# Kotstantinovskiy/SonicDiffusionBayesLab

Measured on AMD Instinct MI355X. Metric: 512x512 images/sec at 50 DDIM steps, higher is better.
Workload: dtype bf16; 1 GPU; SD-1.5 512x512 DDIM 50 steps, CFG 7.5, batch=8/GPU (BASELINE configs[1]); global_batch=8, sample_size=64, parallelism=batch-shard x1, weights=SD-1.5-shaped synthetic seed 1234

## Files before the change

### sonicdiffusionbayeslab_amd/asm_lint.py

```python
from __future__ import annotations

import re
import sys

_REG = re.compile(r'\b([va])\[(\d+):(\d+)\]|\b([va])(\d+)\b')


def regs(tok: str) -> set:
    out = set()
    for m in _REG.finditer(tok):
        if m.group(1):
            out |= {f"{m.group(1)}{i}" for i in range(int(m.group(2)), int(m.group(3)) + 1)}
        else:
            out.add(f"{m.group(4)}{m.group(5)}")
    return out


def kernels(text: str, want: str = ""):
    for m in re.finditer(r'^(\w+):[ \t]*; @\1[^\n]*\n(.*?)^\.Lfunc_end\d+:', text, flags=re.S | re.M):
        if want in m.group(1):
            yield m.group(1), m.group(2)


def _instructions(body: str):
    for line in body.split("\n"):
        mm = re.match(r'^(\.LBB\d+_\d+):', line)
        if mm:
            yield mm.group(1), None
            continue
        t = line.split(";")[0].strip()
        if t and not t.startswith("."):
            yield None, t


def _split_ops(rest: str):
    out, depth, cur = [], 0, ""
    for ch in rest:
        if ch == "[":
            depth += 1
        elif ch == "]":
            depth -= 1
        if ch == "," and depth == 0:
            out.append(cur.strip()); cur = ""
        else:
            cur += ch
    if cur.strip():
        out.append(cur.strip())
    return out


_PASSES = (("v_mfma_f32_16x16x32_bf16", 4), ("v_mfma_f32_16x16x32_f16", 4), ("v_mfma_f32_16x16x32_fp8", 4), ("v_mfma_f32_16x16x32_bf8", 4),
           ("v_mfma_f32_32x32x16_bf16", 8), ("v_mfma_f32_32x32x16_f16", 8), ("v_mfma_f32_32x32x16_fp8", 8), ("v_mfma_f32_32x32x16_bf8", 8),
           ("v_mfma_scale_f32_16x16x128_f8f6f4", 8), ("v_mfma_f32_16x16x128_f8f6f4", 8),
           ("v_mfma_scale_f32_32x32x64_f8f6f4", 16), ("v_mfma_f32_32x32x64_f8f6f4", 16))


def _mfma_passes(op: str) -> int:
    for name, p in _PASSES:
        if op.startswith(name):
            return p
    return 16


def check_pk_opsel(name: str, body: str):
    errs = []
    for _, t in _instructions(body):
        if t and re.match(r'v_pk_\w+_f32\b', t):
            m = re.search(r'op_sel:\[([01,]+)\]', t)
            if m and "1" in m.group(1):
                errs.append(f"{name}: PK_OPSEL `{t}`")
    return errs


def check_store_soffset(name: str, body: str):
    errs = []
    for _, t in _instructions(body):
        if t and re.match(r'buffer_store_(dwordx3|dwordx4|b96|b128|format_xyzw?)\b', t):
            ops = _split_ops(t.split(None, 1)[1])
            soff = ops[3].split()[0] if len(ops) > 3 else "0"
            if re.match(r's\d+|m0|ttmp', soff):
                errs.append(f"{name}: STORE_SOFF `{t}`")
    return errs


def check_mfma_distance(name: str, body: str):
    errs = []
    live = []
    for lab, t in _instructions(body):
        if t is None:
            continue
        op = t.split()[0]
        rest = t.split(None, 1)[1] if " " in t else ""
        if op in ("s_branch", "s_endpgm", "s_setpc_b64"):
            live = []
            continue
        if op == "s_nop":
            n = int(rest.strip()) + 1
            for e in live:
                e[0] += n
            continue
        ops = _split_ops(rest)
        is_mfma = op.startswith("v_mfma") or op.startswith("v_smfmac")
        reads, writes = set(), set()
        if op.startswith("v_") and not is_mfma:
            if op.startswith(("v_cmp", "v_readfirstlane", "v_readlane")):
                for o in ops[1:]:
                    reads |= regs(o)
            elif op.startswith(("v_swap", "v_permlane16_swap", "v_permlane32_swap")):
                for o in ops:
                    reads |= regs(o); writes |= regs(o)
            else:
                writes |= regs(ops[0]) if ops else set()
                for o in ops[1:]:
                    reads |= regs(o)
                if op.startswith(("v_fmac", "v_mac", "v_pk_fmac", "v_dot2c", "v_accvgpr_write")) and ops:
                    reads |= regs(ops[0])
        elif op.startswith(("ds_write", "ds_store", "buffer_store", "global_store", "flat_store", "scratch_store", "buffer_atomic", "global_atomic")):
            for o in ops:
                reads |= regs(o)
        elif op.startswith(("ds_read", "ds_load", "buffer_load", "global_load", "flat_load", "scratch_load", "ds_bpermute", "ds_permute", "ds_swizzle")):
            if ops and " lds" not in (" " + rest):
                writes |= regs(ops[0])
            for o in ops[1:]:
                reads |= regs(o)
            if " lds" in (" " + rest) and ops:
                reads |= regs(ops[0])
        if not is_mfma:
            for ws, p, d, c, mt in live:
                if reads & d and ws < p + 4:
                    errs.append(f"{name}: MFMA_DIST `{t}` reads {sorted(reads & d)[:2]} {ws} wait states after `{mt}` (needs {p + 4})")
                if writes & d and ws < p + 1:
                    errs.append(f"{name}: MFMA_DIST `{t}` writes {sorted(writes & d)[:2]} {ws} wait states after `{mt}` (needs {p + 1})")
                if writes & c and ws < p - 4:
                    errs.append(f"{name}: MFMA_DIST `{t}` writes SrcC {sorted(writes & c)[:2]} {ws} wait states after `{mt}` (needs {p - 4})")
        for e in live:
            e[0] += 1
        live = [e for e in live if e[0] < 24]
        if is_mfma and len(ops) >= 4:
            d = regs(ops[0]); c = regs(ops[3].split()[0]) - d
            live.append([0, _mfma_passes(op), d, c, t])
    return errs


def check_lds_waits(name: str, body: str):
    errors = []
    blocks, cur, lab = [], [], "entry"
    for l, t in _instructions(body):
        if l:
            blocks.append((lab, cur)); cur = []; lab = l
        else:
            cur.append(t)
    blocks.append((lab, cur))
    n_tr = 0
    for lab, ins in blocks:
        pending = []
        has_tr = any(i.startswith("ds_read_b64_tr_b16") for i in ins)
        for k, i in enumerate(ins):
            op = i.split()[0]
            if op.startswith("scratch_"):
                errors.append(f"{name} {lab}: spill instruction `{i}`")
                continue
            if op.startswith("ds_"):
                touched = regs(i.split(None, 1)[1]) if " " in i else set()
                for _, d in pending:
                    if d & touched:
                        errors.append(f"{name} {lab}: `{i}` names {sorted(d & touched)} while an LDS read into it is in flight")
                dest = regs(i.split(None, 1)[1].split(",")[0]) if op.startswith("ds_read") else set()
                pending.append((op, dest))
                n_tr += op == "ds_read_b64_tr_b16"
                continue
            if op.startswith("s_load") or op.startswith("s_buffer_load") or op == "s_memtime":
                if has_tr:
                    errors.append(f"{name} {lab}: scalar-memory instruction `{i}` in a block with counted LDS waits")
                continue
            if op == "s_waitcnt":
                mm = re.search(r'lgkmcnt\((\d+)\)', i)
                if mm:
                    n = int(mm.group(1))
                    pending = pending[len(pending) - n:] if n else []
                elif "vmcnt" not in i and "expcnt" not in i:
                    pending = []
                continue
            touched = regs(i.split(None, 1)[1]) if " " in i else set()
            for o, d in pending:
                if d & touched:
                    errors.append(f"{name} {lab}: `{i}` (instruction {k}) uses {sorted(d & touched)} before the {o} that writes it is waited for")
        if has_tr and any(o == "ds_read_b64_tr_b16" for o, _ in pending):
            errors.append(f"{name} {lab}: block ends with transposed reads still in flight")
    return errors, n_tr


LDS_WAIT_KERNELS = {"attention": ["attn_pipe40_kernel", "attn_pipe80_kernel", "attn_pipe64_kernel"]}


def lint_file(path: str, unit: str | None = None, verbose: bool = True):
    text = open(path).read()
    unit = unit or path.rsplit("/", 1)[-1].split(".")[0]
    bad, nk = [], 0
    for name, body in kernels(text):
        nk += 1
        bad += check_pk_opsel(name, body)
        bad += check_store_soffset(name, body)
        bad += check_mfma_distance(name, body)
    for want in LDS_WAIT_KERNELS.get(unit, []):
        found = 0
        for name, body in kernels(text, want):
            found += 1
            errs, n_tr = check_lds_waits(name, body)
            if verbose:
                print(f"{name}: {n_tr} ds_read_b64_tr_b16, {len(errs)} violation(s)")
            bad += errs
        if not found:
            bad.append(f"no kernel matching {want} in {path}")
    if nk != text.count(".amdhsa_kernel "):
        bad.append(f"{path}: {text.count('.amdhsa_kernel ')} kernel descriptors but {nk} function bodies recognised")
    if verbose:
        print(f"asm_lint {path}: {nk} kernels, {len(bad)} violation(s)")
        for e in bad[:40]:
            print("  VIOLATION:", e)
    return bad


if __name__ == "__main__":
    rc = 0
    for p in sys.argv[1:]:
        rc |= 1 if lint_file(p) else 0
    sys.exit(rc)
```

### sonicdiffusionbayeslab_amd/csrc/attention.hip

```cpp
#include "common.h"
#include "kernels.h"

#include <stdlib.h>

namespace {

__device__ __forceinline__ float half_pair_max(float x) {
    const unsigned a = __builtin_bit_cast(unsigned, x);
    const auto sw = __builtin_amdgcn_permlane32_swap(a, a, false, false);
    const unsigned r0 = sw[0], r1 = sw[1];
    return fmaxf(__builtin_bit_cast(float, r0), __builtin_bit_cast(float, r1));
}

__device__ __forceinline__ int pi_swap23(int r) { return (r & ~12) | ((r & 4) << 1) | ((r & 8) >> 1); }

__device__ __forceinline__ void xcd_work_item(int nq, int heads, int xcd_order, int& qblk, int& head, int& b) {
    const int G = gridDim.x, L = blockIdx.x;
    const int q = G >> 3, r = G & 7, xcd = L & 7, idx = L >> 3;
    const int v = xcd_order ? (xcd < r ? xcd * (q + 1) : r * (q + 1) + (xcd - r) * q) + idx : L;
    qblk = v % nq;
    const int rest = v / nq;
    head = rest % heads;
    b = rest / heads;
}
// ... 496 lines not shown
    for (int j = 0; j < NIW; ++j) {
        const int inst = wave + NW * j;
        d_ptr[j] = zero; d_step[j] = 0;
        if (inst < CHK) {
            const int ch = inst * 64 + lane, key = ch / CHK, part = ch - key * CHK;
            if (part < CD) {
                const long ld = a.kv_head_major ? D : a.ldk;
                const long base = a.kv_head_major ? ((long)b * a.heads + head) * a.Nk * D : (long)b * a.Nk * a.ldk + head * D;
                d_ptr[j] = (const char*)(a.K + base + (long)key * ld + part * 8);
                d_step[j] = 64 * ld * 2;
            }
        } else if (inst < NI) {
            const int ch = (inst - CHK) * 64 + lane, key = ch / CHV, part = ch - key * CHV;
            if (part < CD) {
                const long ld = a.kv_head_major ? D : a.ldv;
                const long base = a.kv_head_major ? ((long)b * a.heads + head) * a.Nk * D : (long)b * a.Nk * a.ldv + head * D;
                d_ptr[j] = (const char*)(a.V + base + (long)key * ld + part * 8);
                d_step[j] = 64 * ld * 2;
            } else if (part == CD) {
                d_ptr[j] = ones;
            }
        } else if (V & 2) {
            d_ptr[j] = ones;
        }
    }
    const int ntiles = a.Nk / 64;
    auto issue = [&](int t) {
        char* base = smem + (t & 3) * TILE;
        const bool real = t < ntiles;
#pragma unroll
        for (int j = 0; j < NIW; ++j) {
            const char* src = real ? d_ptr[j] + d_step[j] * t : zero;
            glds16(src, base + (wave + NW * j) * 1024);
        }
    };
    auto wait_keep = [&](int tiles_in_flight) {
        if (tiles_in_flight == 2) asm volatile("s_waitcnt vmcnt(%0)" ::"n"(2 * NIW) : "memory");
        else if (tiles_in_flight == 1) asm volatile("s_waitcnt vmcnt(%0)" ::"n"(NIW) : "memory");
        else asm volatile("s_waitcnt vmcnt(0)" ::: "memory");
    };

    f32x16 o[DVT];
#pragma unroll
    for (int t = 0; t < DVT; ++t)
#pragma unroll
        for (int i = 0; i < 16; ++i) o[t][i] = 0.f;

    const int kfrag_off = pi_swap23(r) * RSK + h * 16;
    static_assert(KBYTES + 37 * RSV + 2 * CD * 8 + 32 * RSK >= 11 * 1024 && KBYTES + 37 * RSV + 2 * CD * 8 + 32 * RSK + 16 <= 12 * 1024,
                  "second ones chunk inside the padding piece");
    const int kfrag2_off = h ? KBYTES + 37 * RSV + 2 * CD * 8 - 64 : kfrag_off;
    const int g16 = (lane >> 4) & 1, q4 = (lane & 15) >> 2, p4 = lane & 3;
    const int vtr_off = KBYTES + (8 * h + q4) * RSV + (16 * g16 + 4 * p4) * 2;

    auto qk = [&](const char* tile, f32x16& s0, f32x16& s1) {
        const char* kp = tile + kfrag_off;
        bf16x8 kf[2 * KQ];
#pragma unroll
        for (int kk = 0; kk < KQ; ++kk) {
            const char* kpp = ((V & 2) && kk == KQ - 1) ? tile + kfrag2_off : kp;
            kf[kk] = *(const bf16x8*)(kpp + kk * 32);
            kf[KQ + kk] = *(const bf16x8*)(kpp + 32 * RSK + kk * 32);
        }
        s0 = __builtin_amdgcn_mfma_f32_32x32x16_bf16(kf[0], qf[0], f32x16{}, 0, 0, 0);
        s1 = __builtin_amdgcn_mfma_f32_32x32x16_bf16(kf[KQ], qf[0], f32x16{}, 0, 0, 0);
#pragma unroll
        for (int kk = 1; kk < KQ; ++kk) {
            s0 = __builtin_amdgcn_mfma_f32_32x32x16_bf16(kf[kk], qf[kk], s0, 0, 0, 0);
            s1 = __builtin_amdgcn_mfma_f32_32x32x16_bf16(kf[KQ + kk], qf[kk], s1, 0, 0, 0);
        }
    };
    auto tile_max = [&](const f32x16& s0, const f32x16& s1) -> float {
        float tmax = fmaxf(s0[0], s1[0]);
#pragma unroll
        for (int i = 1; i < 16; ++i) tmax = fmaxf(tmax, fmaxf(s0[i], s1[i]));
        return half_pair_max(tmax);
    };
    auto softmax_p = [&](const f32x16& s0, const f32x16& s1, float mc, bf16x8* pf) {
#pragma unroll
        for (int s2 = 0; s2 < 4; ++s2) {
            float p[8];
#pragma unroll
            for (int j = 0; j < 8; ++j) {
                const float sv = s2 < 2 ? s0[8 * s2 + j] : s1[8 * (s2 - 2) + j];
                p[j] = (V & 2) ? __builtin_amdgcn_exp2f(sv) : __builtin_amdgcn_exp2f(__builtin_fmaf(sv, c, -mc));
            }
            u32x4 w = {pack2bf(p[0], p[1]), pack2bf(p[2], p[3]), pack2bf(p[4], p[5]), pack2bf(p[6], p[7])};
            pf[s2] = __builtin_bit_cast(bf16x8, w);
        }
    };
    auto pv = [&](const char* tile, const bf16x8* pf) {
#pragma unroll
        for (int tt = 0; tt < DVT; ++tt) {
#pragma unroll
            for (int s2 = 0; s2 < 4; ++s2) {
                const char* ap = tile + s2 * 16 * RSV + vtr_off + tt * 64;
                const bf16x4 lo = __builtin_amdgcn_ds_read_tr16_b64_v4i16((__attribute__((address_space(3))) bf16x4*)(ap));
                const bf16x4 hi = __builtin_amdgcn_ds_read_tr16_b64_v4i16((__attribute__((address_space(3))) bf16x4*)(ap + 4 * RSV));
                const bf16x8 vf = bf16x8{lo[0], lo[1], lo[2], lo[3], hi[0], hi[1], hi[2], hi[3]};
                o[tt] = __builtin_amdgcn_mfma_f32_32x32x16_bf16(vf, pf[s2], o[tt], 0, 0, 0);
            }
        }
    };

    issue(0);
    issue(1);
    issue(2);
    wait_keep(2);
    __builtin_amdgcn_s_barrier();
    asm volatile("" ::: "memory");
    f32x16 sa0, sa1, sb0, sb1;
    qk(smem, sa0, sa1);
    float m_run = tile_max(sa0, sa1);
    auto set_ref = [&](float m) -> float {
        const unsigned pb = pack2bf(-m, 0.f) & 0xffffu;
        if (h) qf[KQ - 1][0] = (short)pb;
        return -bf2f((bf16_t)pb);
    };
    if (V & 2) {
        m_run = set_ref(m_run);
#pragma unroll
        for (int i = 0; i < 16; ++i) { sa0[i] -= m_run; sa1[i] -= m_run; }
    }
    constexpr float STALE = 8.f;
    const unsigned lds_v = (unsigned)(size_t)(__attribute__((address_space(3))) char*)smem + (unsigned)vtr_off;

    auto exp_group = [&](const f32x16& c0, const f32x16& c1, int s2, float mc) -> bf16x8 {
        float p[8];
        if (V & 2) {
#pragma unroll
            for (int j = 0; j < 8; ++j) p[j] = __builtin_amdgcn_exp2f(s2 < 2 ? c0[8 * s2 + j] : c1[8 * (s2 - 2) + j]);
            u32x4 w = {pack2bf(p[0], p[1]), pack2bf(p[2], p[3]), pack2bf(p[4], p[5]), pack2bf(p[6], p[7])};
            return __builtin_bit_cast(bf16x8, w);
        }
        const f32x2_t cc = {c, c}, mm = {-mc, -mc};
#pragma unroll
        for (int j = 0; j < 8; j += 2) {
            const f32x2_t sv = s2 < 2 ? f32x2_t{c0[8 * s2 + j], c0[8 * s2 + j + 1]}
                                      : f32x2_t{c1[8 * (s2 - 2) + j], c1[8 * (s2 - 2) + j + 1]};
            const f32x2_t e = __builtin_elementwise_fma(sv, cc, mm);
            p[j] = __builtin_amdgcn_exp2f(e[0]);
            p[j + 1] = __builtin_amdgcn_exp2f(e[1]);
        }
        u32x4 w = {pack2bf(p[0], p[1]), pack2bf(p[2], p[3]), pack2bf(p[4], p[5]), pack2bf(p[6], p[7])};
        return __builtin_bit_cast(bf16x8, w);
    };
    auto vfrag = [&](const char* tile, int tt, int s2) -> bf16x8 {
        const char* ap = tile + s2 * 16 * RSV + vtr_off + tt * 64;
        const bf16x4 lo = __builtin_amdgcn_ds_read_tr16_b64_v4i16((__attribute__((address_space(3))) bf16x4*)(ap));
        const bf16x4 hi = __builtin_amdgcn_ds_read_tr16_b64_v4i16((__attribute__((address_space(3))) bf16x4*)(ap + 4 * RSV));
        return bf16x8{lo[0], lo[1], lo[2], lo[3], hi[0], hi[1], hi[2], hi[3]};
    };
    auto steady = [&](int t, f32x16& c0, f32x16& c1, f32x16& n0, f32x16& n1) {
        wait_keep(1);
        __builtin_amdgcn_s_barrier();
        asm volatile("" ::: "memory");
        issue(t + 3);
        const char* cur = smem + (t & 3) * TILE;
        const char* kp = smem + ((t + 1) & 3) * TILE + kfrag_off;
        const char* kp2 = (V & 2) ? smem + ((t + 1) & 3) * TILE + kfrag2_off : kp;
        const float mc = m_run * c;
        bf16x8 kf[2 * KQ];
#pragma unroll
        for (int kk = 0; kk < KQ; ++kk) {
            const char* kpp = kk == KQ - 1 ? kp2 : kp;
            kf[kk] = *(const bf16x8*)(kpp + kk * 32);
            kf[KQ + kk] = *(const bf16x8*)(kpp + 32 * RSK + kk * 32);
        }
        bf16x8 pf[4], va, vb;
        const unsigned vaddr = lds_v + (unsigned)((t & 3) * TILE);
        bf16x4 xal, xah, xbl, xbh, yal, yah, ybl, ybh;
#define SD_VREAD(S, G)                                                                                     \
        SD_TR_READ(S##al, vaddr, (G) * 16 * RSV); SD_TR_READ(S##ah, vaddr, (G) * 16 * RSV + 4 * RSV);      \
        SD_TR_READ(S##bl, vaddr, (G) * 16 * RSV + 64); SD_TR_READ(S##bh, vaddr, (G) * 16 * RSV + 64 + 4 * RSV);
#define SD_VREADY_A(S, N)                                                                                  \
        asm volatile("s_waitcnt lgkmcnt(%2)" : "+v"(S##al), "+v"(S##ah) : "n"(N));                        \
        va = bf16x8{S##al[0], S##al[1], S##al[2], S##al[3], S##ah[0], S##ah[1], S##ah[2], S##ah[3]};
#define SD_VREADY_B(S, N)                                                                                  \
        asm volatile("s_waitcnt lgkmcnt(%3)" : "+v"(S##bl), "+v"(S##bh), "+v"(o[0]) : "n"(N));            \
        vb = bf16x8{S##bl[0], S##bl[1], S##bl[2], S##bl[3], S##bh[0], S##bh[1], S##bh[2], S##bh[3]};
        constexpr bool ASM = V & 1, PING = (V & 5) == 5;
        __builtin_amdgcn_sched_barrier(0);
        n0 = __builtin_amdgcn_mfma_f32_32x32x16_bf16(kf[0], qf[0], f32x16{}, 0, 0, 0);
        n1 = __builtin_amdgcn_mfma_f32_32x32x16_bf16(kf[KQ], qf[0], f32x16{}, 0, 0, 0);
        pf[0] = exp_group(c0, c1, 0, mc);
        __builtin_amdgcn_sched_barrier(0);
        n0 = __builtin_amdgcn_mfma_f32_32x32x16_bf16(kf[1], qf[1], n0, 0, 0, 0);
        n1 = __builtin_amdgcn_mfma_f32_32x32x16_bf16(kf[KQ + 1], qf[1], n1, 0, 0, 0);
        pf[1] = exp_group(c0, c1, 1, mc);
        __builtin_amdgcn_sched_barrier(0);
        if (PING) { SD_VREAD(x, 0) __builtin_amdgcn_sched_barrier(0); }
        n0 = __builtin_amdgcn_mfma_f32_32x32x16_bf16(kf[2], qf[2], n0, 0, 0, 0);
        n1 = __builtin_amdgcn_mfma_f32_32x32x16_bf16(kf[KQ + 2], qf[2], n1, 0, 0, 0);
        pf[2] = exp_group(c0, c1, 2, mc);
        if (!ASM) { va = vfrag(cur, 0, 0); vb = vfrag(cur, 1, 0); }
        else if (!PING) { SD_VREAD(x, 0) }
        __builtin_amdgcn_sched_barrier(0);
        if (PING) { SD_VREAD(y, 1) SD_VREADY_A(x, 6) }
        else if (ASM) { SD_VREADY_A(x, 2) }
        o[0] = __builtin_amdgcn_mfma_f32_32x32x16_bf16(va, pf[0], o[0], 0, 0, 0);
        if (PING) { SD_VREADY_B(x, 4) }
        else if (ASM) { SD_VREADY_B(x, 0) }
        o[1] = __builtin_amdgcn_mfma_f32_32x32x16_bf16(vb, pf[0], o[1], 0, 0, 0);
        pf[3] = exp_group(c0, c1, 3, mc);
        if (!ASM) { va = vfrag(cur, 0, 1); vb = vfrag(cur, 1, 1); }
        else if (!PING) { SD_VREAD(x, 1) }
        __builtin_amdgcn_sched_barrier(0);
        if (PING) { SD_VREAD(x, 2) SD_VREADY_A(y, 6) }
        else if (ASM) { SD_VREADY_A(x, 2) }
        o[0] = __builtin_amdgcn_mfma_f32_32x32x16_bf16(va, pf[1], o[0], 0, 0, 0);
        if (PING) { SD_VREADY_B(y, 4) }
        else if (ASM) { SD_VREADY_B(x, 0) }
        o[1] = __builtin_amdgcn_mfma_f32_32x32x16_bf16(vb, pf[1], o[1], 0, 0, 0);
        float tm0 = fmaxf(n0[0], n1[0]);
#pragma unroll
        for (int i = 1; i < 8; ++i) tm0 = (V & 2) ? fmaxf(fmaxf(tm0, n0[i]), n1[i]) : fmaxf(tm0, fmaxf(n0[i], n1[i]));
        if (!ASM) { va = vfrag(cur, 0, 2); vb = vfrag(cur, 1, 2); }
        else if (!PING) { SD_VREAD(x, 2) }
        __builtin_amdgcn_sched_barrier(0);
        if (PING) { SD_VREAD(y, 3) SD_VREADY_A(x, 6) }
        else if (ASM) { SD_VREADY_A(x, 2) }
        o[0] = __builtin_amdgcn_mfma_f32_32x32x16_bf16(va, pf[2], o[0], 0, 0, 0);
        if (PING) { SD_VREADY_B(x, 4) }
        else if (ASM) { SD_VREADY_B(x, 0) }
        o[1] = __builtin_amdgcn_mfma_f32_32x32x16_bf16(vb, pf[2], o[1], 0, 0, 0);
#pragma unroll
        for (int i = 8; i < 16; ++i) tm0 = (V & 2) ? fmaxf(fmaxf(tm0, n0[i]), n1[i]) : fmaxf(tm0, fmaxf(n0[i], n1[i]));
        if (!ASM) { va = vfrag(cur, 0, 3); vb = vfrag(cur, 1, 3); }
        else if (!PING) { SD_VREAD(x, 3) }
        __builtin_amdgcn_sched_barrier(0);
        if (PING) { SD_VREADY_A(y, 2) }
        else if (ASM) { SD_VREADY_A(x, 2) }
        o[0] = __builtin_amdgcn_mfma_f32_32x32x16_bf16(va, pf[3], o[0], 0, 0, 0);
        if (PING) { SD_VREADY_B(y, 0) }
        else if (ASM) { SD_VREADY_B(x, 0) }
        o[1] = __builtin_amdgcn_mfma_f32_32x32x16_bf16(vb, pf[3], o[1], 0, 0, 0);
        const float tmx = half_pair_max(tm0);
        const float m_new = fmaxf(m_run, tmx);
        __builtin_amdgcn_sched_barrier(0);
        if (V & 2) {
            if (!__all(tmx <= STALE)) {
                const float m_old = m_run;
                m_run = set_ref(m_run + fmaxf(tmx, 0.f));
                const float d = m_run - m_old;
                const float alpha = __builtin_amdgcn_exp2f(-d);
#pragma unroll
                for (int tt = 0; tt < DVT; ++tt)
#pragma unroll
                    for (int i = 0; i < 16; ++i) o[tt][i] *= alpha;
#pragma unroll
                for (int i = 0; i < 16; ++i) { n0[i] -= d; n1[i] -= d; }
            }
        } else if (!__all(m_new == m_run)) {
            const float alpha = __builtin_amdgcn_exp2f((m_run - m_new) * c);
#pragma unroll
            for (int tt = 0; tt < DVT; ++tt)
#pragma unroll
                for (int i = 0; i < 16; ++i) o[tt][i] *= alpha;
            m_run = m_new;
        }
    };
    auto final_tile = [&](int t, f32x16& c0, f32x16& c1) {
        wait_keep(0);
        __builtin_amdgcn_s_barrier();
        asm volatile("" ::: "memory");
        bf16x8 pf[4];
        softmax_p(c0, c1, m_run * c, pf);
        pv(smem + (t & 3) * TILE, pf);
    };
#undef SD_VREAD
#undef SD_VREADY_A
#undef SD_VREADY_B
    int t = 0;
    for (; t + 2 < ntiles; t += 2) {
        steady(t, sa0, sa1, sb0, sb1);
        steady(t + 1, sb0, sb1, sa0, sa1);
    }
    if (t + 2 == ntiles) {
        steady(t, sa0, sa1, sb0, sb1);
        final_tile(t + 1, sb0, sb1);
    } else {
        final_tile(t, sa0, sa1);
    }

    constexpr int TT = D / 32, RR = D % 32, REG = (RR & 3) + 4 * (RR >> 3);
    const float inv = 1.0f / __shfl(o[TT][REG], r);
    if (qvalid) {
        bf16_t* op = a.O + ((long)b * a.Nq + q) * a.ldo + head * D;
#pragma unroll
        for (int tt = 0; tt < DVT; ++tt) {
#pragma unroll
            for (int g4 = 0; g4 < 4; ++g4) {
                const int dv = 32 * tt + 8 * g4 + 4 * h;
                if (dv < D) {
                    u32x2 w = {pack2bf(o[tt][4 * g4 + 0] * inv, o[tt][4 * g4 + 1] * inv),
                               pack2bf(o[tt][4 * g4 + 2] * inv, o[tt][4 * g4 + 3] * inv)};
                    *(u32x2*)(op + dv) = w;
                }
            }
        }
    }
}

int launch_attn_pipe40(const AttnArgs& a, hipStream_t stream) {
    static bool attr_set = false;
    if (!attr_set) {
        SD_CHECK_HIP(hipFuncSetAttribute((const void*)attn_pipe40_kernel<0>, hipFuncAttributeMaxDynamicSharedMemorySize, PipeCfg::SMEM));
        SD_CHECK_HIP(hipFuncSetAttribute((const void*)attn_pipe40_kernel<1>, hipFuncAttributeMaxDynamicSharedMemorySize, PipeCfg::SMEM));
        SD_CHECK_HIP(hipFuncSetAttribute((const void*)attn_pipe40_kernel<7>, hipFuncAttributeMaxDynamicSharedMemorySize, PipeCfg::SMEM));
        SD_CHECK_HIP(hipFuncSetAttribute((const void*)attn_pipe40_kernel<3>, hipFuncAttributeMaxDynamicSharedMemorySize, PipeCfg::SMEM));
        attr_set = true;
    }
    constexpr int QB = PipeCfg::NW * 32;
    SD_REQUIRE((long)((a.Nq + QB - 1) / QB) * a.heads * a.B < (1l << 31), "attention: grid too large");
    dim3 grid(((a.Nq + QB - 1) / QB) * a.heads * a.B);
    static const int variant = getenv("SD_ATTN_VARIANT") ? atoi(getenv("SD_ATTN_VARIANT")) & 7 : 7;
    const dim3 blk(PipeCfg::NW * 64);
    if (variant == 0) hipLaunchKernelGGL(attn_pipe40_kernel<0>, grid, blk, PipeCfg::SMEM, stream, a);
    else if (variant == 1) hipLaunchKernelGGL(attn_pipe40_kernel<1>, grid, blk, PipeCfg::SMEM, stream, a);
    else if (variant == 3) hipLaunchKernelGGL(attn_pipe40_kernel<3>, grid, blk, PipeCfg::SMEM, stream, a);
    else hipLaunchKernelGGL(attn_pipe40_kernel<7>, grid, blk, PipeCfg::SMEM, stream, a);
    SD_CHECK_HIP(hipGetLastError());
    return 0;
}

struct Pipe80Cfg {
    static constexpr int D = 80, KQ = 5, DVT = 3, CD = 10, CHK = 11, CHV = 12, RSK = 176, RSV = 192;
    static constexpr int KBYTES = 64 * RSK, NI = CHK + CHV, NW = 4;
    static constexpr int NIW = 6;
    static constexpr int VBYTES = 64 * RSV, NSLOT = 3;
    static constexpr int VOFF = NSLOT * KBYTES, PADOFF = VOFF + NSLOT * VBYTES;
    static constexpr int SMEM = PADOFF + 1024 + 256;
    static_assert(KBYTES == CHK * 1024 && VBYTES == CHV * 1024 && SMEM <= 80 * 1024, "whole DMA pieces; two workgroups per CU");
};

__global__ __launch_bounds__(Pipe80Cfg::NW * 64, 2) void attn_pipe80_kernel(const AttnArgs a) {
    using Cfg = Pipe80Cfg;
    constexpr int D = Cfg::D, KQ = Cfg::KQ, DVT = Cfg::DVT, CD = Cfg::CD, CHK = Cfg::CHK, CHV = Cfg::CHV;
    constexpr int RSK = Cfg::RSK, RSV = Cfg::RSV, KBYTES = Cfg::KBYTES, VBYTES = Cfg::VBYTES, NI = Cfg::NI, NIW = Cfg::NIW;
    constexpr int NW = Cfg::NW, VOFF = Cfg::VOFF, PADOFF = Cfg::PADOFF;

    extern __shared__ __attribute__((aligned(16))) char smem[];
    const int tid = threadIdx.x, lane = tid & 63;
    const int wave = __builtin_amdgcn_readfirstlane(tid >> 6);
    const int r = lane & 31, h = lane >> 5;
    int qblk, head, b;
    xcd_work_item((a.Nq + NW * 32 - 1) / (NW * 32), a.heads, a.xcd_order, qblk, head, b);
    const int q = qblk * (NW * 32) + wave * 32 + r;
    const bool qvalid = q < a.Nq;
    const float c = a.q_prescaled ? 1.0f : a.scale * 1.4426950408889634f;
    const char* zero = (const char*)a.consts;
    const char* ones = zero + 256;

    bf16x8 qf[KQ];
    {
        const bf16_t* qp = a.Q + ((long)b * a.Nq + (qvalid ? q : 0)) * a.ldq + head * D;
#pragma unroll
        for (int kk = 0; kk < KQ; ++kk) {
            if (qvalid) qf[kk] = *(const bf16x8*)(qp + kk * 16 + h * 8);
            else qf[kk] = bf16x8{0, 0, 0, 0, 0, 0, 0, 0};
        }
#pragma unroll
        for (int kk = 0; kk < KQ; ++kk) asm volatile("" : "+v"(qf[kk]));
    }

    const char* d_ptr[NIW];
    long d_step[NIW];
#pragma unroll
    for (int j = 0; j < NIW; ++j) {
        const int inst = wave + NW * j;
        d_ptr[j] = zero; d_step[j] = 0;
        if (inst < CHK) {
            const int ch = inst * 64 + lane, key = ch / CHK, part = ch - key * CHK;
            if (part < CD) {
                d_ptr[j] = (const char*)(a.K + (long)b * a.Nk * a.ldk + head * D + (long)key * a.ldk + part * 8);
                d_step[j] = 64 * a.ldk * 2;
            }
        } else if (inst < NI) {
            const int ch = (inst - CHK) * 64 + lane, key = ch / CHV, part = ch - key * CHV;
            if (part < CD) {
                d_ptr[j] = (const char*)(a.V + (long)b * a.Nk * a.ldv + head * D + (long)key * a.ldv + part * 8);
                d_step[j] = 64 * a.ldv * 2;
            } else if (part == CD) {
                d_ptr[j] = ones;
            }
        }
    }
    const int ntiles = a.Nk / 64;
    auto issue = [&](int tk, int ks, int tv, int vs) {
#pragma unroll
        for (int j = 0; j < NIW; ++j) {
            const int inst = wave + NW * j;
            const bool isk = inst < CHK;
            const int t = isk ? tk : tv;
            const char* src = t < ntiles ? d_ptr[j] + d_step[j] * t : zero;
            char* dst = isk ? smem + ks * KBYTES + inst * 1024 : inst < NI ? smem + VOFF + vs * VBYTES + (inst - CHK) * 1024 : smem + PADOFF;
            glds16(src, dst);
        }
    };

    f32x16 o[DVT];
#pragma unroll
    for (int t = 0; t < DVT; ++t)
#pragma unroll
        for (int i = 0; i < 16; ++i) o[t][i] = 0.f;

    const int kfrag_off = pi_swap23(r) * RSK + h * 16;
    const int g16 = (lane >> 4) & 1, q4 = (lane & 15) >> 2, p4 = lane & 3;
    const int vtr_off = VOFF + (8 * h + q4) * RSV + (16 * g16 + 4 * p4) * 2;
    const unsigned lds_v = (unsigned)(size_t)(__attribute__((address_space(3))) char*)smem + (unsigned)vtr_off;

    auto qk = [&](const char* tile, f32x16& s0, f32x16& s1) {
        const char* kp = tile + kfrag_off;
        s0 = __builtin_amdgcn_mfma_f32_32x32x16_bf16(*(const bf16x8*)(kp), qf[0], f32x16{}, 0, 0, 0);
        s1 = __builtin_amdgcn_mfma_f32_32x32x16_bf16(*(const bf16x8*)(kp + 32 * RSK), qf[0], f32x16{}, 0, 0, 0);
#pragma unroll
        for (int kk = 1; kk < KQ; ++kk) {
            s0 = __builtin_amdgcn_mfma_f32_32x32x16_bf16(*(const bf16x8*)(kp + kk * 32), qf[kk], s0, 0, 0, 0);
            s1 = __builtin_amdgcn_mfma_f32_32x32x16_bf16(*(const bf16x8*)(kp + 32 * RSK + kk * 32), qf[kk], s1, 0, 0, 0);
        }
    };
    auto exp_group = [&](const f32x16& c0, const f32x16& c1, int s2, float mc) -> bf16x8 {
        float p[8];
#pragma unroll
        for (int j = 0; j < 8; ++j) p[j] = __builtin_amdgcn_exp2f(__builtin_fmaf(s2 < 2 ? c0[8 * s2 + j] : c1[8 * (s2 - 2) + j], c, -mc));
        u32x4 w = {pack2bf(p[0], p[1]), pack2bf(p[2], p[3]), pack2bf(p[4], p[5]), pack2bf(p[6], p[7])};
        return __builtin_bit_cast(bf16x8, w);
    };

    issue(0, 0, 0, 0);
    issue(1, 1, 0, 0);
    issue(2, 2, 1, 1);
    asm volatile("s_waitcnt vmcnt(%0)" ::"n"(2 * NIW) : "memory");
    __builtin_amdgcn_s_barrier();
    asm volatile("" ::: "memory");
    f32x16 sa0, sa1, sb0, sb1;
    qk(smem, sa0, sa1);
    float m_run;
    {
        float tm = fmaxf(sa0[0], sa1[0]);
#pragma unroll
        for (int i = 1; i < 16; ++i) tm = fmaxf(fmaxf(tm, sa0[i]), sa1[i]);
        m_run = half_pair_max(tm);
    }
    constexpr float STALE = 8.f;

#define SD_VREAD80(S, G)                                                                                    \
    SD_TR_READ(S##0l, vaddr, (G) * 16 * RSV); SD_TR_READ(S##0h, vaddr, (G) * 16 * RSV + 4 * RSV);           \
    SD_TR_READ(S##1l, vaddr, (G) * 16 * RSV + 64); SD_TR_READ(S##1h, vaddr, (G) * 16 * RSV + 64 + 4 * RSV); \
    SD_TR_READ(S##2l, vaddr, (G) * 16 * RSV + 128); SD_TR_READ(S##2h, vaddr, (G) * 16 * RSV + 128 + 4 * RSV);
#define SD_VREADY80(S, N)                                                                                   \
    asm volatile("s_waitcnt lgkmcnt(%6)" : "+v"(S##0l), "+v"(S##0h), "+v"(S##1l), "+v"(S##1h), "+v"(S##2l), "+v"(S##2h) : "n"(N)); \
    v0 = bf16x8{S##0l[0], S##0l[1], S##0l[2], S##0l[3], S##0h[0], S##0h[1], S##0h[2], S##0h[3]};            \
    v1 = bf16x8{S##1l[0], S##1l[1], S##1l[2], S##1l[3], S##1h[0], S##1h[1], S##1h[2], S##1h[3]};            \
    v2 = bf16x8{S##2l[0], S##2l[1], S##2l[2], S##2l[3], S##2h[0], S##2h[1], S##2h[2], S##2h[3]};
#define SD_PV80(G)                                                                                          \
    o[0] = __builtin_amdgcn_mfma_f32_32x32x16_bf16(v0, pf[G], o[0], 0, 0, 0);                               \
    o[1] = __builtin_amdgcn_mfma_f32_32x32x16_bf16(v1, pf[G], o[1], 0, 0, 0);                               \
    o[2] = __builtin_amdgcn_mfma_f32_32x32x16_bf16(v2, pf[G], o[2], 0, 0, 0);

    auto steady = [&](int t, int slot, f32x16& c0, f32x16& c1, f32x16& n0, f32x16& n1) {
        asm volatile("s_waitcnt vmcnt(%0)" ::"n"(NIW) : "memory");
        __builtin_amdgcn_s_barrier();
        asm volatile("" ::: "memory");
        const int nslot = slot == 2 ? 0 : slot + 1, fslot = slot == 0 ? 2 : slot - 1;
        issue(t + 3, slot, t + 2, fslot);
        const char* kp = smem + nslot * KBYTES + kfrag_off;
        const float mc = m_run * c;
        bf16x8 kf[2 * KQ];
#pragma unroll
        for (int kk = 0; kk < KQ; ++kk) {
            kf[kk] = *(const bf16x8*)(kp + kk * 32);
            kf[KQ + kk] = *(const bf16x8*)(kp + 32 * RSK + kk * 32);
        }
        bf16x8 pf[4], v0, v1, v2;
        const unsigned vaddr = lds_v + (unsigned)(slot * VBYTES);
        bf16x4 x0l, x0h, x1l, x1h, x2l, x2h, y0l, y0h, y1l, y1h, y2l, y2h;
        __builtin_amdgcn_sched_barrier(0);
        n0 = __builtin_amdgcn_mfma_f32_32x32x16_bf16(kf[0], qf[0], f32x16{}, 0, 0, 0);
        n1 = __builtin_amdgcn_mfma_f32_32x32x16_bf16(kf[KQ], qf[0], f32x16{}, 0, 0, 0);
        pf[0] = exp_group(c0, c1, 0, mc);
        __builtin_amdgcn_sched_barrier(0);
        n0 = __builtin_amdgcn_mfma_f32_32x32x16_bf16(kf[1], qf[1], n0, 0, 0, 0);
        n1 = __builtin_amdgcn_mfma_f32_32x32x16_bf16(kf[KQ + 1], qf[1], n1, 0, 0, 0);
        pf[1] = exp_group(c0, c1, 1, mc);
        __builtin_amdgcn_sched_barrier(0);
        n0 = __builtin_amdgcn_mfma_f32_32x32x16_bf16(kf[2], qf[2], n0, 0, 0, 0);
        n1 = __builtin_amdgcn_mfma_f32_32x32x16_bf16(kf[KQ + 2], qf[2], n1, 0, 0, 0);
        pf[2] = exp_group(c0, c1, 2, mc);
        __builtin_amdgcn_sched_barrier(0);
        n0 = __builtin_amdgcn_mfma_f32_32x32x16_bf16(kf[3], qf[3], n0, 0, 0, 0);
        n1 = __builtin_amdgcn_mfma_f32_32x32x16_bf16(kf[KQ + 3], qf[3], n1, 0, 0, 0);
        pf[3] = exp_group(c0, c1, 3, mc);
        __builtin_amdgcn_sched_barrier(0);
        SD_VREAD80(x, 0)
        __builtin_amdgcn_sched_barrier(0);
        n0 = __builtin_amdgcn_mfma_f32_32x32x16_bf16(kf[4], qf[4], n0, 0, 0, 0);
        n1 = __builtin_amdgcn_mfma_f32_32x32x16_bf16(kf[KQ + 4], qf[4], n1, 0, 0, 0);
        __builtin_amdgcn_sched_barrier(0);
        SD_VREAD80(y, 1) SD_VREADY80(x, 6)
        SD_PV80(0)
        float tm0 = fmaxf(n0[0], n1[0]);
#pragma unroll
        for (int i = 1; i < 4; ++i) tm0 = fmaxf(fmaxf(tm0, n0[i]), n1[i]);
        __builtin_amdgcn_sched_barrier(0);
        SD_VREAD80(x, 2) SD_VREADY80(y, 6)
        SD_PV80(1)
#pragma unroll
        for (int i = 4; i < 8; ++i) tm0 = fmaxf(fmaxf(tm0, n0[i]), n1[i]);
        __builtin_amdgcn_sched_barrier(0);
        SD_VREAD80(y, 3) SD_VREADY80(x, 6)
        SD_PV80(2)
#pragma unroll
        for (int i = 8; i < 12; ++i) tm0 = fmaxf(fmaxf(tm0, n0[i]), n1[i]);
        __builtin_amdgcn_sched_barrier(0);
        SD_VREADY80(y, 0)
        SD_PV80(3)
#pragma unroll
        for (int i = 12; i < 16; ++i) tm0 = fmaxf(fmaxf(tm0, n0[i]), n1[i]);
        const float tmx = half_pair_max(tm0);
        __builtin_amdgcn_sched_barrier(0);
        if (!__all((tmx - m_run) * c <= STALE)) {
            const float m_new = fmaxf(m_run, tmx);
            const float alpha = __builtin_amdgcn_exp2f((m_run - m_new) * c);
#pragma unroll
            for (int tt = 0; tt < DVT; ++tt)
#pragma unroll
                for (int i = 0; i < 16; ++i) o[tt][i] *= alpha;
            m_run = m_new;
        }
    };
    auto final_tile = [&](int slot, f32x16& c0, f32x16& c1) {
        asm volatile("s_waitcnt vmcnt(0)" ::: "memory");
        __builtin_amdgcn_s_barrier();
        asm volatile("" ::: "memory");
        const float mc = m_run * c;
        bf16x8 pf[4], v0, v1, v2;
#pragma unroll
        for (int s2 = 0; s2 < 4; ++s2) pf[s2] = exp_group(c0, c1, s2, mc);
        const unsigned vaddr = lds_v + (unsigned)(slot * VBYTES);
        bf16x4 x0l, x0h, x1l, x1h, x2l, x2h;
        __builtin_amdgcn_sched_barrier(0);
        SD_VREAD80(x, 0) SD_VREADY80(x, 0) SD_PV80(0)
        __builtin_amdgcn_sched_barrier(0);
        SD_VREAD80(x, 1) SD_VREADY80(x, 0) SD_PV80(1)
        __builtin_amdgcn_sched_barrier(0);
        SD_VREAD80(x, 2) SD_VREADY80(x, 0) SD_PV80(2)
        __builtin_amdgcn_sched_barrier(0);
        SD_VREAD80(x, 3) SD_VREADY80(x, 0) SD_PV80(3)
        __builtin_amdgcn_sched_barrier(0);
    };
#undef SD_VREAD80
#undef SD_VREADY80
#undef SD_PV80
    int t = 0, slot = 0;
    for (; t + 2 < ntiles; t += 2) {
        steady(t, slot, sa0, sa1, sb0, sb1);
        slot = slot == 2 ? 0 : slot + 1;
        steady(t + 1, slot, sb0, sb1, sa0, sa1);
        slot = slot == 2 ? 0 : slot + 1;
    }
    if (t + 2 == ntiles) {
        steady(t, slot, sa0, sa1, sb0, sb1);
        slot = slot == 2 ? 0 : slot + 1;
        final_tile(slot, sb0, sb1);
    } else {
        final_tile(slot, sa0, sa1);
    }

    constexpr int TT = D / 32, RR = D % 32, REG = (RR & 3) + 4 * (RR >> 3);
    static_assert((RR & 4) == 0, "ones row must sit in the h = 0 half");
    const float inv = 1.0f / __shfl(o[TT][REG], r);
    if (qvalid) {
        bf16_t* op = a.O + ((long)b * a.Nq + q) * a.ldo + head * D;
#pragma unroll
        for (int tt = 0; tt < DVT; ++tt) {
#pragma unroll
            for (int g4 = 0; g4 < 4; ++g4) {
                const int dv = 32 * tt + 8 * g4 + 4 * h;
                if (dv < D) {
                    u32x2 w = {pack2bf(o[tt][4 * g4 + 0] * inv, o[tt][4 * g4 + 1] * inv),
                               pack2bf(o[tt][4 * g4 + 2] * inv, o[tt][4 * g4 + 3] * inv)};
                    *(u32x2*)(op + dv) = w;
                }
            }
        }
    }
}

int launch_attn_pipe80(const AttnArgs& a, hipStream_t stream) {
    static bool attr_set = false;
    if (!attr_set) {
        SD_CHECK_HIP(hipFuncSetAttribute((const void*)attn_pipe80_kernel, hipFuncAttributeMaxDynamicSharedMemorySize, Pipe80Cfg::SMEM));
        attr_set = true;
    }
    constexpr int QB = Pipe80Cfg::NW * 32;
    SD_REQUIRE((long)((a.Nq + QB - 1) / QB) * a.heads * a.B < (1l << 31), "attention: grid too large");
    dim3 grid(((a.Nq + QB - 1) / QB) * a.heads * a.B);
    hipLaunchKernelGGL(attn_pipe80_kernel, grid, dim3(Pipe80Cfg::NW * 64), Pipe80Cfg::SMEM, stream, a);
    SD_CHECK_HIP(hipGetLastError());
    return 0;
}

template <bool ONES>
struct Pipe64Cfg {
    static constexpr int D = 64, KQ = 4, DVT = ONES ? 3 : 2, CD = 8, CHK = 9, CHV = ONES ? 12 : 9, RSK = 144, RSV = CHV * 16;
    static constexpr int KBYTES = 64 * RSK, NI = CHK + CHV, NW = 4;
    static constexpr int NIW = (NI + NW - 1) / NW;
    static constexpr int VBYTES = 64 * RSV, NSLOT = 3;
    static constexpr int VOFF = NSLOT * KBYTES, PADOFF = VOFF + NSLOT * VBYTES;
    static constexpr int SMEM = PADOFF + 1024 + 256;
    static constexpr int RPS = 2 * DVT;
    static_assert(KBYTES == CHK * 1024 && VBYTES == CHV * 1024 && SMEM <= 80 * 1024, "whole DMA pieces; two workgroups per CU");
};

template <bool ONES>
__global__ __launch_bounds__(Pipe64Cfg<ONES>::NW * 64, 2) void attn_pipe64_kernel(const AttnArgs a) {
    using Cfg = Pipe64Cfg<ONES>;
    constexpr int D = Cfg::D, KQ = Cfg::KQ, DVT = Cfg::DVT, CD = Cfg::CD, CHK = Cfg::CHK, CHV = Cfg::CHV;
    constexpr int RSK = Cfg::RSK, RSV = Cfg::RSV, KBYTES = Cfg::KBYTES, VBYTES = Cfg::VBYTES, NI = Cfg::NI, NIW = Cfg::NIW;
// ... 358 lines not shown
```

Before: 11.17 images/s.

## Add two-strand D=40 attention kernel processing 64 queries per wave

Adds a variant of the head-dim-40 flash attention kernel in which each wave handles two 32-query strands. Each K/V tile loaded into LDS serves twice as many queries, and the QK, exp and PV stages of the two strands are interleaved to hide MFMA and transcendental latency. It becomes the default when the grid has enough work items. The cost is higher register pressure, half as many workgroups, and a more complex schedule.

After: 11.24 images/s (median of 6 runs). No clear change (+0.6%).

```diff
diff --git a/sonicdiffusionbayeslab_amd/asm_lint.py b/sonicdiffusionbayeslab_amd/asm_lint.py
--- a/sonicdiffusionbayeslab_amd/asm_lint.py
+++ b/sonicdiffusionbayeslab_amd/asm_lint.py
@@ -190,7 +190,7 @@
     return errors, n_tr
 
 
-LDS_WAIT_KERNELS = {"attention": ["attn_pipe40_kernel", "attn_pipe80_kernel", "attn_pipe64_kernel"]}
+LDS_WAIT_KERNELS = {"attention": ["attn_pipe40_kernel", "attn_pipe40s2_kernel", "attn_pipe80_kernel", "attn_pipe64_kernel"]}
 
 
 def lint_file(path: str, unit: str | None = None, verbose: bool = True):
diff --git a/sonicdiffusionbayeslab_amd/csrc/attention.hip b/sonicdiffusionbayeslab_amd/csrc/attention.hip
--- a/sonicdiffusionbayeslab_amd/csrc/attention.hip
+++ b/sonicdiffusionbayeslab_amd/csrc/attention.hip
@@ -822,9 +822,330 @@
     }
 }
 
+__global__ __launch_bounds__(PipeCfg::NW * 64, 2) void attn_pipe40s2_kernel(const AttnArgs a) {
+    using Cfg = PipeCfg;
+    constexpr int D = Cfg::D, KQ = Cfg::KQ, DVT = Cfg::DVT, CD = Cfg::CD, CHK = Cfg::CHK, CHV = Cfg::CHV;
+    constexpr int RSK = Cfg::RSK, RSV = Cfg::RSV, KBYTES = Cfg::KBYTES, TILE = Cfg::TILE, NI = Cfg::NI, NIW = Cfg::NIW;
+    constexpr int NW = Cfg::NW, QB = NW * 64;
+
+    extern __shared__ __attribute__((aligned(16))) char smem[];
+    const int tid = threadIdx.x, lane = tid & 63;
+    const int wave = __builtin_amdgcn_readfirstlane(tid >> 6);
+    const int r = lane & 31, h = lane >> 5;
+    int qblk, head, b;
+    xcd_work_item(a.Nq / QB, a.heads, a.xcd_order, qblk, head, b);
+    const int q = qblk * QB + wave * 64 + r;
+    const float c = a.q_prescaled ? 1.0f : a.scale * 1.4426950408889634f;
+    const char* zero = (const char*)a.consts;
+    const char* ones = zero + 256;
+
+    bf16x8 qf0[KQ], qf1[KQ];
+    auto load_q = [&](int qq, bf16x8* qf) {
+        const bf16_t* qp = a.Q + ((long)b * a.Nq + qq) * a.ldq + head * D;
+#pragma unroll
+        for (int kk = 0; kk < KQ; ++kk) {
+            const int col = kk * 16 + h * 8;
+            if (col < D) qf[kk] = *(const bf16x8*)(qp + col);
+            else qf[kk] = bf16x8{0, 0, 0, 0, 0, 0, 0, 0};
+        }
+        if (!a.q_prescaled) {
+#pragma unroll
+            for (int kk = 0; kk < KQ; ++kk) {
+                u32x4 w;
+#pragma unroll
+                for (int j = 0; j < 4; ++j)
+                    w[j] = pack2bf(bf2f((bf16_t)qf[kk][2 * j]) * c, bf2f((bf16_t)qf[kk][2 * j + 1]) * c);
+                qf[kk] = __builtin_bit_cast(bf16x8, w);
+            }
+        }
+#pragma unroll
+        for (int kk = 0; kk < KQ; ++kk) asm volatile("" : "+v"(qf[kk]));
+    };
+    load_q(q, qf0);
+    load_q(q + 32, qf1);
+
+    const char* d_ptr[NIW];
+    unsigned d_step[NIW];
+#pragma unroll
+    for (int j = 0; j < NIW; ++j) {
+        const int inst = wave + NW * j;
+        d_ptr[j] = zero; d_step[j] = 0;
+        if (inst < CHK) {
+            const int ch = inst * 64 + lane, key = ch / CHK, part = ch - key * CHK;
+            if (part < CD) {
+                const long ld = a.kv_head_major ? D : a.ldk;
+                const long base = a.kv_head_major ? ((long)b * a.heads + head) * a.Nk * D : (long)b * a.Nk * a.ldk + head * D;
+                d_ptr[j] = (const char*)(a.K + base + (long)key * ld + part * 8);
+                d_step[j] = (unsigned)(64 * ld * 2);
+            }
+        } else if (inst < NI) {
+            const int ch = (inst - CHK) * 64 + lane, key = ch / CHV, part = ch - key * CHV;
+            if (part < CD) {
+                const long ld = a.kv_head_major ? D : a.ldv;
+                const long base = a.kv_head_major ? ((long)b * a.heads + head) * a.Nk * D : (long)b * a.Nk * a.ldv + head * D;
+                d_ptr[j] = (const char*)(a.V + base + (long)key * ld + part * 8);
+                d_step[j] = (unsigned)(64 * ld * 2);
+            } else if (part == CD) {
+                d_ptr[j] = ones;
+            }
+        } else {
+            d_ptr[j] = ones;
+        }
+    }
+    const int ntiles = a.Nk / 64;
+    auto issue = [&](int t) {
+        char* base = smem + (t & 3) * TILE;
+        const bool real = t < ntiles;
+#pragma unroll
+        for (int j = 0; j < NIW; ++j) {
+            glds16(real ? d_ptr[j] : zero, base + (wave + NW * j) * 1024);
+            d_ptr[j] += d_step[j];
+        }
+    };
+    auto wait_keep = [&](int tiles_in_flight) {
+        if (tiles_in_flight == 2) asm volatile("s_waitcnt vmcnt(%0)" ::"n"(2 * NIW) : "memory");
+        else if (tiles_in_flight == 1) asm volatile("s_waitcnt vmcnt(%0)" ::"n"(NIW) : "memory");
+        else asm volatile("s_waitcnt vmcnt(0)" ::: "memory");
+    };
+
+    f32x16 o0[DVT], o1[DVT];
+#pragma unroll
+    for (int t = 0; t < DVT; ++t)
+#pragma unroll
+        for (int i = 0; i < 16; ++i) { o0[t][i] = 0.f; o1[t][i] = 0.f; }
+
+    const int kfrag_off = pi_swap23(r) * RSK + h * 16;
+    const int kfrag2_off = h ? KBYTES + 37 * RSV + 2 * CD * 8 - 64 : kfrag_off;
+    const int g16 = (lane >> 4) & 1, q4 = (lane & 15) >> 2, p4 = lane & 3;
+    const int vtr_off = KBYTES + (8 * h + q4) * RSV + (16 * g16 + 4 * p4) * 2;
+
+    auto kfrags = [&](const char* tile, bf16x8* kf) {
+#pragma unroll
+        for (int kk = 0; kk < KQ; ++kk) {
+            const char* kpp = tile + (kk == KQ - 1 ? kfrag2_off : kfrag_off);
+            kf[kk] = *(const bf16x8*)(kpp + kk * 32);
+            kf[KQ + kk] = *(const bf16x8*)(kpp + 32 * RSK + kk * 32);
+        }
+    };
+    auto tile_max = [&](const f32x16& s0, const f32x16& s1) -> float {
+        float tmax = fmaxf(s0[0], s1[0]);
+#pragma unroll
+        for (int i = 1; i < 16; ++i) tmax = fmaxf(tmax, fmaxf(s0[i], s1[i]));
+        return half_pair_max(tmax);
+    };
+    auto exp_group = [&](const f32x16& c0, const f32x16& c1, int s2) -> bf16x8 {
+        float p[8];
+#pragma unroll
+        for (int j = 0; j < 8; ++j) p[j] = __builtin_amdgcn_exp2f(s2 < 2 ? c0[8 * s2 + j] : c1[8 * (s2 - 2) + j]);
+        u32x4 w = {pack2bf(p[0], p[1]), pack2bf(p[2], p[3]), pack2bf(p[4], p[5]), pack2bf(p[6], p[7])};
+        return __builtin_bit_cast(bf16x8, w);
+    };
+    auto set_ref = [&](bf16x8* qf, float m) -> float {
+        const unsigned pb = pack2bf(-m, 0.f) & 0xffffu;
+        if (h) qf[KQ - 1][0] = (short)pb;
+        return -bf2f((bf16_t)pb);
+    };
+
+    issue(0);
+    issue(1);
+    issue(2);
+    wait_keep(2);
+    __builtin_amdgcn_s_barrier();
+    asm volatile("" ::: "memory");
+    f32x16 x0, x1;
+    f32x16 y0, y1, z0, z1;
+    {
+        bf16x8 kf[2 * KQ];
+        kfrags(smem, kf);
+        x0 = __builtin_amdgcn_mfma_f32_32x32x16_bf16(kf[0], qf0[0], f32x16{}, 0, 0, 0);
+        x1 = __builtin_amdgcn_mfma_f32_32x32x16_bf16(kf[KQ], qf0[0], f32x16{}, 0, 0, 0);
+        y0 = __builtin_amdgcn_mfma_f32_32x32x16_bf16(kf[0], qf1[0], f32x16{}, 0, 0, 0);
+        y1 = __builtin_amdgcn_mfma_f32_32x32x16_bf16(kf[KQ], qf1[0], f32x16{}, 0, 0, 0);
+#pragma unroll
+        for (int kk = 1; kk < KQ; ++kk) {
+            x0 = __builtin_amdgcn_mfma_f32_32x32x16_bf16(kf[kk], qf0[kk], x0, 0, 0, 0);
+            x1 = __builtin_amdgcn_mfma_f32_32x32x16_bf16(kf[KQ + kk], qf0[kk], x1, 0, 0, 0);
+            y0 = __builtin_amdgcn_mfma_f32_32x32x16_bf16(kf[kk], qf1[kk], y0, 0, 0, 0);
+            y1 = __builtin_amdgcn_mfma_f32_32x32x16_bf16(kf[KQ + kk], qf1[kk], y1, 0, 0, 0);
+        }
+    }
+    float m_run0 = set_ref(qf0, tile_max(x0, x1));
+    float m_run1 = set_ref(qf1, tile_max(y0, y1));
+#pragma unroll
+    for (int i = 0; i < 16; ++i) { x0[i] -= m_run0; x1[i] -= m_run0; y0[i] -= m_run1; y1[i] -= m_run1; }
+    constexpr float STALE = 8.f;
+    const unsigned lds_v = (unsigned)(size_t)(__attribute__((address_space(3))) char*)smem + (unsigned)vtr_off;
+
+    auto rescale = [&](float tmx, float& m_run, bf16x8* qf, f32x16* o, f32x16& n0, f32x16& n1) {
+        if (!__all(tmx <= STALE)) {
+            const float m_old = m_run;
+            m_run = set_ref(qf, m_run + fmaxf(tmx, 0.f));
+            const float d = m_run - m_old;
+            const float alpha = __builtin_amdgcn_exp2f(-d);
+#pragma unroll
+            for (int tt = 0; tt < DVT; ++tt)
+#pragma unroll
+                for (int i = 0; i < 16; ++i) o[tt][i] *= alpha;
+#pragma unroll
+            for (int i = 0; i < 16; ++i) { n0[i] -= d; n1[i] -= d; }
+        }
+    };
+
+#define SD_VREAD_A(G, DEP)                                                                                                 \
+    asm volatile("ds_read_b64_tr_b16 %0, %2 offset:%3" : "=v"(val), "+v"(DEP) : "v"(vaddr), "n"((G) * 16 * RSV));          \
+    SD_TR_READ(vah, vaddr, (G) * 16 * RSV + 4 * RSV);
+#define SD_VREAD_B(G, DEP)                                                                                                 \
+    asm volatile("ds_read_b64_tr_b16 %0, %2 offset:%3" : "=v"(vbl), "+v"(DEP) : "v"(vaddr), "n"((G) * 16 * RSV + 64));     \
+    SD_TR_READ(vbh, vaddr, (G) * 16 * RSV + 64 + 4 * RSV);
+#define SD_VREADY_A(N)                                                                                                     \
+    asm volatile("s_waitcnt lgkmcnt(%2)" : "+v"(val), "+v"(vah) : "n"(N));                                                 \
+    va = bf16x8{val[0], val[1], val[2], val[3], vah[0], vah[1], vah[2], vah[3]};
+#define SD_VREADY_B(N, DEP)                                                                                                \
+    asm volatile("s_waitcnt lgkmcnt(%3)" : "+v"(vbl), "+v"(vbh), "+v"(DEP) : "n"(N));                                      \
+    vb = bf16x8{vbl[0], vbl[1], vbl[2], vbl[3], vbh[0], vbh[1], vbh[2], vbh[3]};
+#define SD_PV_GROUP(G, NEXT, NB)                                                                                           \
+    SD_VREADY_A(2)                                                                                                         \
+    o0[0] = __builtin_amdgcn_mfma_f32_32x32x16_bf16(va, pf0[G], o0[0], 0, 0, 0);                                           \
+    o1[0] = __builtin_amdgcn_mfma_f32_32x32x16_bf16(va, pf1[G], o1[0], 0, 0, 0);                                           \
+    if (NEXT) { SD_VREAD_A((G) + 1, o1[0]) }                                                                               \
+    SD_VREADY_B(NB, o1[0])                                                                                                 \
+    o0[1] = __builtin_amdgcn_mfma_f32_32x32x16_bf16(vb, pf0[G], o0[1], 0, 0, 0);                                           \
+    o1[1] = __builtin_amdgcn_mfma_f32_32x32x16_bf16(vb, pf1[G], o1[1], 0, 0, 0);                                           \
+    if (NEXT) { SD_VREAD_B((G) + 1, o1[1]) }
+
+    auto steady = [&](int t, f32x16& c0, f32x16& c1, f32x16& n0, f32x16& n1) {
+        wait_keep(1);
+        __builtin_amdgcn_s_barrier();
+        asm volatile("" ::: "memory");
+        issue(t + 3);
+        bf16x8 kf[2 * KQ];
+        kfrags(smem + ((t + 1) & 3) * TILE, kf);
+        bf16x8 pf0[4], pf1[4], va, vb;
+        bf16x4 val, vah, vbl, vbh;
+        const unsigned vaddr = lds_v + (unsigned)((t & 3) * TILE);
+        __builtin_amdgcn_sched_barrier(0);
+        n0 = __builtin_amdgcn_mfma_f32_32x32x16_bf16(kf[0], qf1[0], f32x16{}, 0, 0, 0);
+        n1 = __builtin_amdgcn_mfma_f32_32x32x16_bf16(kf[KQ], qf1[0], f32x16{}, 0, 0, 0);
+        pf0[0] = exp_group(x0, x1, 0);
+        __builtin_amdgcn_sched_barrier(0);
+        n0 = __builtin_amdgcn_mfma_f32_32x32x16_bf16(kf[1], qf1[1], n0, 0, 0, 0);
+        n1 = __builtin_amdgcn_mfma_f32_32x32x16_bf16(kf[KQ + 1], qf1[1], n1, 0, 0, 0);
+        pf0[1] = exp_group(x0, x1, 1);
+        __builtin_amdgcn_sched_barrier(0);
+        n0 = __builtin_amdgcn_mfma_f32_32x32x16_bf16(kf[2], qf1[2], n0, 0, 0, 0);
+        n1 = __builtin_amdgcn_mfma_f32_32x32x16_bf16(kf[KQ + 2], qf1[2], n1, 0, 0, 0);
+        pf0[2] = exp_group(x0, x1, 2);
+        pf0[3] = exp_group(x0, x1, 3);
+        __builtin_amdgcn_sched_barrier(0);
+        x0 = __builtin_amdgcn_mfma_f32_32x32x16_bf16(kf[0], qf0[0], f32x16{}, 0, 0, 0);
+        pf1[0] = exp_group(c0, c1, 0);
+        x0 = __builtin_amdgcn_mfma_f32_32x32x16_bf16(kf[1], qf0[1], x0, 0, 0, 0);
+        __builtin_amdgcn_sched_barrier(0);
+        x0 = __builtin_amdgcn_mfma_f32_32x32x16_bf16(kf[2], qf0[2], x0, 0, 0, 0);
+        pf1[1] = exp_group(c0, c1, 1);
+        x1 = __builtin_amdgcn_mfma_f32_32x32x16_bf16(kf[KQ], qf0[0], f32x16{}, 0, 0, 0);
+        __builtin_amdgcn_sched_barrier(0);
+        SD_VREAD_A(0, o1[0])
+        SD_VREAD_B(0, o1[1])
+        __builtin_amdgcn_sched_barrier(0);
+        x1 = __builtin_amdgcn_mfma_f32_32x32x16_bf16(kf[KQ + 1], qf0[1], x1, 0, 0, 0);
+        x1 = __builtin_amdgcn_mfma_f32_32x32x16_bf16(kf[KQ + 2], qf0[2], x1, 0, 0, 0);
+        float tm1 = fmaxf(n0[0], n1[0]);
+#pragma unroll
+        for (int i = 1; i < 8; ++i) tm1 = fmaxf(fmaxf(tm1, n0[i]), n1[i]);
+        __builtin_amdgcn_sched_barrier(0);
+        SD_PV_GROUP(0, true, 2)
+        pf1[2] = exp_group(c0, c1, 2);
+        __builtin_amdgcn_sched_barrier(0);
+        SD_PV_GROUP(1, true, 2)
+        pf1[3] = exp_group(c0, c1, 3);
+        __builtin_amdgcn_sched_barrier(0);
+        SD_PV_GROUP(2, true, 2)
+#pragma unroll
+        for (int i = 8; i < 16; ++i) tm1 = fmaxf(fmaxf(tm1, n0[i]), n1[i]);
+        float tm0 = fmaxf(x0[0], x1[0]);
+#pragma unroll
+        for (int i = 1; i < 8; ++i) tm0 = fmaxf(fmaxf(tm0, x0[i]), x1[i]);
+        __builtin_amdgcn_sched_barrier(0);
+        SD_PV_GROUP(3, false, 0)
+#pragma unroll
+        for (int i = 8; i < 16; ++i) tm0 = fmaxf(fmaxf(tm0, x0[i]), x1[i]);
+        const float tmx0 = half_pair_max(tm0);
+        const float tmx1 = half_pair_max(tm1);
+        __builtin_amdgcn_sched_barrier(0);
+        rescale(tmx0, m_run0, qf0, o0, x0, x1);
+        rescale(tmx1, m_run1, qf1, o1, n0, n1);
+    };
+#undef SD_PV_GROUP
+#undef SD_VREAD_A
+#undef SD_VREAD_B
+#undef SD_VREADY_A
+#undef SD_VREADY_B
+    auto final_tile = [&](int t, const f32x16& c0, const f32x16& c1, int vtr_off_e) {
+        wait_keep(0);
+        __builtin_amdgcn_s_barrier();
+        asm volatile("" ::: "memory");
+        const char* tile = smem + (t & 3) * TILE;
+        bf16x8 pf0[4], pf1[4];
+#pragma unroll
+        for (int s2 = 0; s2 < 4; ++s2) { pf0[s2] = exp_group(x0, x1, s2); pf1[s2] = exp_group(c0, c1, s2); }
+#pragma unroll
+        for (int tt = 0; tt < DVT; ++tt) {
+#pragma unroll
+            for (int s2 = 0; s2 < 4; ++s2) {
+                const char* ap = tile + s2 * 16 * RSV + vtr_off_e + tt * 64;
+                const bf16x4 lo = __builtin_amdgcn_ds_read_tr16_b64_v4i16((__attribute__((address_space(3))) bf16x4*)(ap));
+                const bf16x4 hi = __builtin_amdgcn_ds_read_tr16_b64_v4i16((__attribute__((address_space(3))) bf16x4*)(ap + 4 * RSV));
+                const bf16x8 vf = bf16x8{lo[0], lo[1], lo[2], lo[3], hi[0], hi[1], hi[2], hi[3]};
+                o0[tt] = __builtin_amdgcn_mfma_f32_32x32x16_bf16(vf, pf0[s2], o0[tt], 0, 0, 0);
+                o1[tt] = __builtin_amdgcn_mfma_f32_32x32x16_bf16(vf, pf1[s2], o1[tt], 0, 0, 0);
+            }
+        }
+    };
+    int t = 0;
+    for (; t + 2 < ntiles; t += 2) {
+        steady(t, y0, y1, z0, z1);
+        steady(t + 1, z0, z1, y0, y1);
+    }
+    const bool one_more = t + 2 == ntiles;
+    if (one_more) steady(t, y0, y1, z0, z1);
+    int lane_e = __builtin_amdgcn_mbcnt_hi(~0u, __builtin_amdgcn_mbcnt_lo(~0u, 0u));
+    asm volatile("" : "+v"(lane_e));
+    const int r_e = lane_e & 31, h_e = lane_e >> 5;
+    const int vtr_off_e = KBYTES + (8 * h_e + ((lane_e & 15) >> 2)) * RSV + (16 * ((lane_e >> 4) & 1) + 4 * (lane_e & 3)) * 2;
+    const int q_e = qblk * QB + wave * 64 + r_e;
+    if (one_more) final_tile(t + 1, z0, z1, vtr_off_e);
+    else final_tile(t, y0, y1, vtr_off_e);
+
+    constexpr int TT = D / 32, RR = D % 32, REG = (RR & 3) + 4 * (RR >> 3);
+    auto store = [&](int qq, const f32x16* o) {
+        const int h = h_e;
+        const float inv = 1.0f / __shfl(o[TT][REG], r_e);
+        bf16_t* op = a.O + ((long)b * a.Nq + qq) * a.ldo + head * D;
+#pragma unroll
+        for (int tt = 0; tt < DVT; ++tt) {
+#pragma unroll
+            for (int g4 = 0; g4 < 4; ++g4) {
+                const int dv = 32 * tt + 8 * g4 + 4 * h;
+                if (dv < D) {
+                    u32x2 w = {pack2bf(o[tt][4 * g4 + 0] * inv, o[tt][4 * g4 + 1] * inv),
+                               pack2bf(o[tt][4 * g4 + 2] * inv, o[tt][4 * g4 + 3] * inv)};
+                    *(u32x2*)(op + dv) = w;
+                }
+            }
+        }
+    };
+    store(q_e, o0);
+    store(q_e + 32, o1);
+}
+
+constexpr int STRANDS_MIN_ITEMS = 512;
+constexpr bool STRANDS_DEFAULT = true;
+
 int launch_attn_pipe40(const AttnArgs& a, hipStream_t stream) {
     static bool attr_set = false;
     if (!attr_set) {
+        SD_CHECK_HIP(hipFuncSetAttribute((const void*)attn_pipe40s2_kernel, hipFuncAttributeMaxDynamicSharedMemorySize, PipeCfg::SMEM));
         SD_CHECK_HIP(hipFuncSetAttribute((const void*)attn_pipe40_kernel<0>, hipFuncAttributeMaxDynamicSharedMemorySize, PipeCfg::SMEM));
         SD_CHECK_HIP(hipFuncSetAttribute((const void*)attn_pipe40_kernel<1>, hipFuncAttributeMaxDynamicSharedMemorySize, PipeCfg::SMEM));
         SD_CHECK_HIP(hipFuncSetAttribute((const void*)attn_pipe40_kernel<7>, hipFuncAttributeMaxDynamicSharedMemorySize, PipeCfg::SMEM));
@@ -836,6 +1157,16 @@
     dim3 grid(((a.Nq + QB - 1) / QB) * a.heads * a.B);
     static const int variant = getenv("SD_ATTN_VARIANT") ? atoi(getenv("SD_ATTN_VARIANT")) & 7 : 7;
     const dim3 blk(PipeCfg::NW * 64);
+    if (variant == 7 && a.Nq % (2 * QB) == 0 && a.ldk < (1l << 24) && a.ldv < (1l << 24)) {
+        const char* e = getenv("SD_ATTN_STRANDS");
+        const int strands = e ? atoi(e) : 0;
+        const long items = (long)(a.Nq / (2 * QB)) * a.heads * a.B;
+        if (strands == 2 || (strands != 1 && STRANDS_DEFAULT && items >= STRANDS_MIN_ITEMS)) {
+            hipLaunchKernelGGL(attn_pipe40s2_kernel, dim3((unsigned)items), blk, PipeCfg::SMEM, stream, a);
+            SD_CHECK_HIP(hipGetLastError());
+            return 0;
+        }
+    }
     if (variant == 0) hipLaunchKernelGGL(attn_pipe40_kernel<0>, grid, blk, PipeCfg::SMEM, stream, a);
     else if (variant == 1) hipLaunchKernelGGL(attn_pipe40_kernel<1>, grid, blk, PipeCfg::SMEM, stream, a);
     else if (variant == 3) hipLaunchKernelGGL(attn_pipe40_kernel<3>, grid, blk, PipeCfg::SMEM, stream, a);
```
